# snphbaum/scikit-gpuppy

Hardware: AMD Instinct MI355X
Metric: GP fit+predict pts/sec (K+Cholesky, N=16384 d=8) (higher is better)
Workload: dtype f64; 1 GPU; C3: N=16384 d=8 M=16384 fit(Gram+Cholesky+alpha)+estimate_many, theta fixed; global_batch=32768, parallelism=1 GPU

## Files before the change

### scikit-gpuppy_amd/csrc/emu.hip

```cpp
#include <math.h>
#include <stdint.h>
#include <stdlib.h>
#include <algorithm>

#include "common.h"

#include "gemm_tile.h"

typedef int v4i __attribute__((ext_vector_type(4)));
typedef int v16i __attribute__((ext_vector_type(16)));

constexpr int EMU_MAXL = 16;
constexpr int EMU_BT = 256;
constexpr int EMU_BK = 128;

constexpr int EMU_MODULI[EMU_MAXL] = {256, 255, 253, 251, 247, 241, 239, 233, 229, 227, 223, 211, 199, 197, 193, 191};

struct EmuGarner { float c[EMU_MAXL][EMU_MAXL]; };
constexpr EmuGarner emu_garner_table()
{
    EmuGarner g{};
    for (int k = 0; k < EMU_MAXL; ++k)
        for (int j = 0; j < k; ++j) {
            const int pk = EMU_MODULI[k], a = EMU_MODULI[j] % pk;
            int inv = 0;
            for (int x = 1; x < pk; ++x)
                if (a * x % pk == 1) { inv = x; break; }
            g.c[j][k] = (float)inv;
        }
    return g;
}
static __constant__ const int emu_p[EMU_MAXL] = {256, 255, 253, 251, 247, 241, 239, 233, 229, 227, 223, 211, 199, 197, 193, 191};
static __constant__ const EmuGarner emu_garner = emu_garner_table();

constexpr int EMU_NONFINITE = 0x7fffffff;

int emu_moduli()
{
    static const int v = [] { const char *e = getenv("GPX_EMU_MODULI"); const int l = e ? atoi(e) : EMU_MAXL; return std::min(EMU_MAXL, std::max(2, l)); }();
    return v;
}
bool emu_enabled(int64_t K)
{
    static const int on = [] { const char *e = getenv("GPX_EMU_F64"); return e ? atoi(e) : 1; }();
    static const long min_k = [] { const char *e = getenv("GPX_EMU_MIN_K"); return e ? atol(e) : 4096L; }();
    return on && K >= min_k && K < (1 << 17) && K % EMU_BK == 0;
}
int emu_scale_bits(int64_t K, int L)
{
    double log2p = 0.0;
    for (int l = 0; l < L; ++l) log2p += log2((double)EMU_MODULI[l]);
    return (int)floor(log2p - 1.0 - log2((double)K) - 1e-9);
}

__global__ __launch_bounds__(256) void emu_split_kernel(const double *__restrict__ X, long ldx, long rows_real, int K, int bits, int L,
                                                        int8_t *__restrict__ res, long plane, int *__restrict__ sig)
{
    const long row = blockIdx.x;
    const int t = threadIdx.x;
    __shared__ double red_max[4];
    __shared__ int red_bad[4];
    int8_t *out = res + row * (long)K;
    if (row >= rows_real) {
        for (int c = 4 * t; c < K; c += 1024)
            for (int l = 0; l < L; ++l) *reinterpret_cast<int *>(out + l * plane + c) = 0;
        if (t == 0) sig[row] = 0;
        return;
    }
    const double *x = X + row * ldx;
    double m = 0.0;
    int bad = 0;
    for (int c = 2 * t; c < K; c += 512) {
        const v2d v = *reinterpret_cast<const v2d *>(x + c);
        bad |= (int)!isfinite(v.x) | (int)!isfinite(v.y);
        m = fmax(m, fmax(fabs(v.x), fabs(v.y)));
    }
#pragma unroll
    for (int o = 32; o > 0; o >>= 1) { m = fmax(m, __shfl_xor(m, o)); bad |= __shfl_xor(bad, o); }
    if ((t & 63) == 0) { red_max[t >> 6] = m; red_bad[t >> 6] = bad; }
    __syncthreads();
    m = fmax(fmax(red_max[0], red_max[1]), fmax(red_max[2], red_max[3]));
    bad = red_bad[0] | red_bad[1] | red_bad[2] | red_bad[3];
    const int s = (bad || m == 0.0) ? 0 : bits - 1 - ilogb(m);
    if (t == 0) sig[row] = bad ? EMU_NONFINITE : s;
    for (int c = 4 * t; c < K; c += 1024) {
        const v2d v0 = *reinterpret_cast<const v2d *>(x + c), v1 = *reinterpret_cast<const v2d *>(x + c + 2);
        double a[4] = {rint(ldexp(v0.x, s)), rint(ldexp(v0.y, s)), rint(ldexp(v1.x, s)), rint(ldexp(v1.y, s))};
        if (bad) a[0] = a[1] = a[2] = a[3] = 0.0;
#pragma unroll
        for (int l = 0; l < EMU_MAXL; ++l) {
            if (l >= L) continue;
            const double p = (double)emu_p[l], pinv = 1.0 / p, h = 0.5 * p;
            unsigned packed = 0;
#pragma unroll
            for (int e = 0; e < 4; ++e) {
                double r = fma(-rint(a[e] * pinv), p, a[e]);
                r = r > h ? r - p : (r < -h ? r + p : r);
                packed |= ((unsigned)(int)r & 0xffu) << (8 * e);
            }
            *reinterpret_cast<unsigned *>(out + l * plane + c) = packed;
        }
    }
}

__global__ __launch_bounds__(512, 1) void emu_i8_gemm_kernel(const int8_t *__restrict__ A, const int8_t *__restrict__ B, long sa, long sb, int K,
                                                             int8_t *__restrict__ R, long ldr, long sr, int tm, int tn)
{
    __shared__ __attribute__((aligned(1024))) int8_t smem[2 * 2 * EMU_BT * EMU_BK];
    constexpr int STAGE = 2 * EMU_BT * EMU_BK;
    const int nwg = gridDim.x, orig = blockIdx.x;
    const int lid = xcd_chunk_start(nwg, orig & 7) + (orig >> 3);
    const int per = tm * tn, z = lid / per;
    int rem = lid - z * per;
    const int g = rem / (8 * tn), first = 8 * g, grows = std::min(8, tm - first);
    rem -= g * 8 * tn;
    const int bx = rem / grows, by = first + rem - bx * grows;

    const int t = threadIdx.x;
    const int wave = __builtin_amdgcn_readfirstlane(t >> 6), lane = t & 63;
    const int wr = wave >> 2, wc = wave & 3;
    const int drow = lane >> 3;
    const char *Abase = reinterpret_cast<const char *>(A + z * sa + (long)by * EMU_BT * K);
    const char *Bbase = reinterpret_cast<const char *>(B + z * sb + (long)bx * EMU_BT * K);
    unsigned off[4];
#pragma unroll
    for (int u = 0; u < 4; ++u) {
        const int row = 8 * (wave + 8 * u) + drow;
        off[u] = (unsigned)((long)row * K + 16 * ((lane & 7) ^ ((row >> 1) & 7)));
    }
    const unsigned lds_base = (unsigned)(unsigned long)(__attribute__((address_space(3))) int8_t *)smem;
#define EMU_DMA_ONE(SBASE, VOFF, LDSBYTES) \
    asm volatile("s_mov_b32 m0, %0\n\ts_nop 0\n\tglobal_load_lds_dwordx4 %1, %2" ::"s"(LDSBYTES), "v"(VOFF), "s"(SBASE) : "memory");
#define EMU_DMA_STAGE(BUF, KT)                                                                                              \
    {                                                                                                                       \
        const char *ak_ = gpx_uniform_ptr(Abase + (long)(KT) * EMU_BK);                                                     \
        const char *bk_ = gpx_uniform_ptr(Bbase + (long)(KT) * EMU_BK);                                                     \
        _Pragma("unroll") for (int u_ = 0; u_ < 4; ++u_)                                                                    \
            EMU_DMA_ONE(ak_, off[u_], __builtin_amdgcn_readfirstlane(lds_base + (unsigned)((BUF) * STAGE + (wave + 8 * u_) * 1024)))  \
        _Pragma("unroll") for (int u_ = 0; u_ < 4; ++u_)                                                                    \
            EMU_DMA_ONE(bk_, off[u_], __builtin_amdgcn_readfirstlane(lds_base + (unsigned)((BUF) * STAGE + EMU_BT * EMU_BK + (wave + 8 * u_) * 1024))) \
    }
    const int nk = K / EMU_BK;
    EMU_DMA_STAGE(0, 0)
    v16i acc[4][2];
#pragma unroll
    for (int i = 0; i < 4; ++i)
#pragma unroll
        for (int j = 0; j < 2; ++j) acc[i][j] = (v16i){};
    asm volatile("s_waitcnt vmcnt(0)" ::: "memory");
    __syncthreads();

    const int fr = lane & 31, sw = (fr >> 1) & 7;
    int koff[4];
#pragma unroll
    for (int kk = 0; kk < 4; ++kk) koff[kk] = 16 * ((2 * kk + (lane >> 5)) ^ sw);
    const int a_row = (wr * 128 + fr) * EMU_BK, b_row = EMU_BT * EMU_BK + (wc * 64 + fr) * EMU_BK;
    typedef const __attribute__((address_space(3))) v4i lds_v4i;
    const __attribute__((address_space(3))) int8_t *lsm = (const __attribute__((address_space(3))) int8_t *)smem;
    v4i fa[2][4], fb[2][2];
#define EMU_LOAD_FRAGS(SET, BUFOFF, KK)                                                              \
    _Pragma("unroll") for (int i_ = 0; i_ < 4; ++i_)                                                 \
        fa[SET][i_] = *(lds_v4i *)(lsm + (BUFOFF) + a_row + i_ * 32 * EMU_BK + koff[KK]);            \
    _Pragma("unroll") for (int i_ = 0; i_ < 2; ++i_)                                                 \
        fb[SET][i_] = *(lds_v4i *)(lsm + (BUFOFF) + b_row + i_ * 32 * EMU_BK + koff[KK]);
#define EMU_MMA(SET)                                                                                 \
    _Pragma("unroll") for (int i_ = 0; i_ < 4; ++i_)                                                 \
        _Pragma("unroll") for (int j_ = 0; j_ < 2; ++j_)                                             \
            acc[i_][j_] = __builtin_amdgcn_mfma_i32_32x32x32_i8(fa[SET][i_], fb[SET][j_], acc[i_][j_], 0, 0, 0);
    EMU_LOAD_FRAGS(0, 0, 0)
#define EMU_KSTEP(CUR_OFF, NXT_OFF, NXT_BUF, KT)                   \
    {                                                             \
        const bool has_next_ = (KT) + 1 < nk;                     \
        if (has_next_) EMU_DMA_STAGE(NXT_BUF, (KT) + 1)           \
        EMU_LOAD_FRAGS(1, CUR_OFF, 1)                             \
        EMU_MMA(0)                                                \
        __builtin_amdgcn_sched_barrier(0);                        \
        EMU_LOAD_FRAGS(0, CUR_OFF, 2)                             \
        EMU_MMA(1)                                                \
        __builtin_amdgcn_sched_barrier(0);                        \
        EMU_LOAD_FRAGS(1, CUR_OFF, 3)                             \
        EMU_MMA(0)                                                \
        __builtin_amdgcn_sched_barrier(0);                        \
        asm volatile("s_waitcnt vmcnt(0)" ::: "memory");          \
        __syncthreads();                                          \
        if (has_next_) { EMU_LOAD_FRAGS(0, NXT_OFF, 0) }          \
        EMU_MMA(1)                                                \
        __builtin_amdgcn_sched_barrier(0);                        \
    }
    for (int kt = 0; kt < nk; kt += 2) {
        EMU_KSTEP(0, STAGE, 1, kt)
        if (kt + 1 < nk) EMU_KSTEP(STAGE, 0, 0, kt + 1)
    }
#undef EMU_KSTEP
#undef EMU_LOAD_FRAGS
#undef EMU_MMA
#undef EMU_DMA_STAGE
#undef EMU_DMA_ONE

    const double p = (double)emu_p[z], pinv = 1.0 / p;
    int8_t *Rw = R + z * sr + ((long)by * EMU_BT + wr * 128 + 4 * (lane >> 5)) * ldr + (long)bx * EMU_BT + wc * 64 + fr;
#pragma unroll
    for (int i = 0; i < 4; ++i)
#pragma unroll
        for (int j = 0; j < 2; ++j)
#pragma unroll
            for (int r = 0; r < 16; ++r) {
                const double v = (double)acc[i][j][r];
                Rw[(long)(i * 32 + (r & 3) + 8 * (r >> 2)) * ldr + j * 32] = (int8_t)(int)fma(-rint(v * pinv), p, v);
            }
}

__global__ __launch_bounds__(256) void emu_rebuild_kernel(const int8_t *__restrict__ R, long ldr, long sr, int L, const int *__restrict__ sa,
                                                          const int *__restrict__ sb, double *__restrict__ C, long ldc, long rows, long cols)
{
    const long q4 = (cols + 3) >> 2;
    const long idx = (long)blockIdx.x * 256 + threadIdx.x;
    const long i = idx / q4, j0 = (idx - i * q4) * 4;
    if (i >= rows) return;
    unsigned w[EMU_MAXL];
#pragma unroll
    for (int l = 0; l < EMU_MAXL; ++l)
        if (l < L) w[l] = *reinterpret_cast<const unsigned *>(R + l * sr + i * ldr + j0);
    const int si = sa[i];
    double *c = C + i * ldc + j0;
#pragma unroll
    for (int e = 0; e < 4; ++e) {
        if (j0 + e >= cols) continue;
        const int tj = sb[j0 + e];
        if (si == EMU_NONFINITE || tj == EMU_NONFINITE) { c[e] = __builtin_nan(""); continue; }
        float v[EMU_MAXL];
        v[0] = (float)(int8_t)(w[0] >> (8 * e));
#pragma unroll
        for (int k = 1; k < EMU_MAXL; ++k) {
            if (k >= L) continue;
            const float pk = (float)emu_p[k], pkinv = 1.0f / pk, hk = 0.5f * (pk - 1.0f);
            float tk = (float)(int8_t)(w[k] >> (8 * e));
#pragma unroll
            for (int jj = 0; jj < k; ++jj) {
                tk = (tk - v[jj]) * emu_garner.c[jj][k];
                tk = fmaf(-rintf(tk * pkinv), pk, tk);
            }
            tk = tk > hk ? tk - pk : (tk < -hk ? tk + pk : tk);
            v[k] = tk;
        }
        __int128 X = (__int128)(int)v[L - 1];
#pragma unroll
        for (int k = EMU_MAXL - 2; k >= 0; --k)
            if (k <= L - 2) X = X * emu_p[k] + (int)v[k];
        const long hi = (long)(X >> 64);
        const unsigned long lo = (unsigned long)X;
        const double xd = (hi == ((long)lo >> 63)) ? (double)(long)lo : fma((double)hi, 0x1p64, (double)lo);
        c[e] -= ldexp(xd, -(si + tj));
    }
}

static int64_t emu_cap(int64_t K, int L) { return std::max<int64_t>(EMU_BT, (((int64_t)1 << 31) / (K * L)) / EMU_BT * EMU_BT); }

void emu_work_need(EmuWork &w, int64_t rows, int64_t cols, int64_t K)
{
    const int L = emu_moduli();
    const int64_t cap = emu_cap(K, L), rt = std::min(round_up(rows, EMU_BT), cap), ct = std::min(round_up(cols, EMU_BT), cap);
    w.a_bytes = std::max(w.a_bytes, rt * K * L);
    w.b_bytes = std::max(w.b_bytes, ct * K * L);
    w.r_bytes = std::max(w.r_bytes, std::min(rt * ct * L, (int64_t)1 << 31));
    w.sig_n = std::max(w.sig_n, rt + ct);
}

int emu_work_alloc(EmuWork &w)
{
    double *a = nullptr, *b = nullptr, *r = nullptr, *g = nullptr;
    int rc = 0;
    if ((rc = dalloc(&a, w.a_bytes / 8)) || (rc = dalloc(&b, w.b_bytes / 8)) || (rc = dalloc(&r, w.r_bytes / 8)) || (rc = dalloc(&g, (w.sig_n + 1) / 2))) {
        if (a) dfree(a);
        if (b) dfree(b);
        if (r) dfree(r);
        return rc;
    }
    w.ra = (int8_t *)a;
    w.rb = (int8_t *)b;
    w.rr = (int8_t *)r;
    w.sig = (int *)g;
    return 0;
}

void emu_work_free(EmuWork &w)
{
    if (w.ra) dfree(w.ra);
    if (w.rb) dfree(w.rb);
    if (w.rr) dfree(w.rr);
    if (w.sig) dfree(w.sig);
    w = EmuWork();
}

static int emu_check_args(const double *A, int64_t lda, const double *B, int64_t ldb, int64_t ldc, int64_t cols, int64_t K)
{
    if (K <= 0 || K % EMU_BK || K >= (1 << 17)) {
        gpx_set_error("emu_gemm_nt_sub: K = %ld is not a multiple of %d in [%d, 2^17)", (long)K, EMU_BK, EMU_BK);
        return GPX_ERR_BAD_ARG;
    }
    if (lda < K || ldb < K || ldc < cols) {
        gpx_set_error("emu_gemm_nt_sub: leading dimension shorter than a row (lda %ld, ldb %ld < K %ld, or ldc %ld < cols %ld)", (long)lda, (long)ldb,
                      (long)K, (long)ldc, (long)cols);
        return GPX_ERR_BAD_ARG;
    }
    if ((lda | ldb) & 1 || ((uintptr_t)A | (uintptr_t)B) & 15) {
        gpx_set_error("emu_gemm_nt_sub: A and B must be 16-byte aligned with even lda, ldb (lda %ld, ldb %ld, A %p, B %p)", (long)lda, (long)ldb,
                      (const void *)A, (const void *)B);
        return GPX_ERR_BAD_ARG;
    }
    return 0;
}

int emu_gemm_nt_sub(const double *A, int64_t lda, const double *B, int64_t ldb, double *C, int64_t ldc, int64_t rows, int64_t cols, int64_t K,
                    const EmuWork &w, hipStream_t s, Profiler *prof)
{
    if (rows <= 0 || cols <= 0) return 0;
    if (K % EMU_BK || K >= (1 << 17)) { gpx_set_error("emu_gemm_nt_sub: K = %ld out of range", (long)K); return GPX_ERR_BAD_ARG; }
    const int L = emu_moduli();
    const int bits = emu_scale_bits(K, L), abits = bits - bits / 2, bbits = bits / 2;
    const int64_t cap = emu_cap(K, L);
    const int64_t rt = std::min<int64_t>(round_up(rows, EMU_BT), cap);
    int64_t ct = std::min<int64_t>(round_up(cols, EMU_BT), cap);
    while (ct > EMU_BT && rt * ct * L > ((int64_t)1 << 31)) ct -= EMU_BT;
    if (!w.ra || rt * K * L > w.a_bytes || ct * K * L > w.b_bytes || rt * ct * L > w.r_bytes || rt + ct > w.sig_n) {
        gpx_set_error("emu_gemm_nt_sub: workspace too small for %ld x %ld x %ld", (long)rows, (long)cols, (long)K);
        return GPX_ERR_STATE;
    }
    ProfScope ps(prof, s, GPX_K_GEMM_EMU, 2.0 * (double)rows * (double)cols * (double)K);
    int8_t *ra = w.ra, *rb = w.rb, *rr = w.rr;
    int *sga = w.sig, *sgb = sga + rt;
    for (int64_t r0 = 0; r0 < rows; r0 += rt) {
        const int64_t nr = std::min(rt, rows - r0), nrp = round_up(nr, EMU_BT);
        hipLaunchKernelGGL(emu_split_kernel, dim3((unsigned)nrp), dim3(256), 0, s, A + r0 * lda, (long)lda, (long)nr, (int)K, abits, L, ra,
                           (long)(nrp * K), sga);
        for (int64_t c0 = 0; c0 < cols; c0 += ct) {
            const int64_t nc = std::min(ct, cols - c0), ncp = round_up(nc, EMU_BT);
            hipLaunchKernelGGL(emu_split_kernel, dim3((unsigned)ncp), dim3(256), 0, s, B + c0 * ldb, (long)ldb, (long)nc, (int)K, bbits, L, rb,
                               (long)(ncp * K), sgb);
            const int tm = (int)(nrp / EMU_BT), tn = (int)(ncp / EMU_BT);
            hipLaunchKernelGGL(emu_i8_gemm_kernel, dim3((unsigned)(tm * tn * L)), dim3(512), 0, s, (const int8_t *)ra, (const int8_t *)rb,
                               (long)(nrp * K), (long)(ncp * K), (int)K, rr, (long)ncp, (long)(nrp * ncp), tm, tn);
            const long thr = (long)nr * ((nc + 3) / 4);
            hipLaunchKernelGGL(emu_rebuild_kernel, dim3((unsigned)((thr + 255) / 256)), dim3(256), 0, s, (const int8_t *)rr, (long)ncp,
                               (long)(nrp * ncp), L, (const int *)sga, (const int *)sgb, C + r0 * ldc + c0, (long)ldc, (long)nr, (long)nc);
        }
        GPX_HIP(hipGetLastError());
    }
    return 0;
}

extern "C" int gpx_emu_gemm_nt_sub(const double *A, int64_t lda, const double *B, int64_t ldb, double *C, int64_t ldc, int64_t rows, int64_t cols,
                                   int64_t K)
{
    GPX_TRY(gpx_require_device());
    if (rows < 0 || cols < 0 || !A || !B || !C) { gpx_set_error("gpx_emu_gemm_nt_sub: bad arguments"); return GPX_ERR_BAD_ARG; }
    GPX_TRY(emu_check_args(A, lda, B, ldb, ldc, cols, K));
    if (rows == 0 || cols == 0) return 0;
    EmuWork w;
    emu_work_need(w, rows, cols, K);
    GPX_TRY(emu_work_alloc(w));
    int rc = emu_gemm_nt_sub(A, lda, B, ldb, C, ldc, rows, cols, K, w, 0, nullptr);
    if (hipStreamSynchronize(0) != hipSuccess && rc == 0) { gpx_set_error("gpx_emu_gemm_nt_sub: stream failed"); rc = GPX_ERR_HIP; }
    emu_work_free(w);
    return rc;
}

__global__ void emu_fill_kernel(int8_t *p, long n, unsigned seed)
{
    for (long i = (long)blockIdx.x * 256 + threadIdx.x; i < n; i += (long)gridDim.x * 256) {
        unsigned x = (unsigned)i * 2654435761u ^ seed;
        x ^= x >> 15; x *= 2246822519u; x ^= x >> 13;
        p[i] = (int8_t)(x & 0xff);
    }
}

extern "C" int gpx_bench_emu_i8(int64_t rows, int64_t cols, int64_t K, int nmod, int iters, double *ms)
{
    GPX_TRY(gpx_require_device());
    if (rows % EMU_BT || cols % EMU_BT || K % EMU_BK || K >= (1 << 17) || nmod < 1 || nmod > EMU_MAXL || iters < 1 || !ms) {
        gpx_set_error("gpx_bench_emu_i8: bad arguments");
        return GPX_ERR_BAD_ARG;
    }
    double *wa = nullptr, *wb = nullptr, *wr = nullptr;
    int rc = 0;
    if ((rc = dalloc(&wa, rows * K * nmod / 8)) || (rc = dalloc(&wb, cols * K * nmod / 8)) || (rc = dalloc(&wr, rows * cols * nmod / 8))) {
        if (wa) dfree(wa);
        if (wb) dfree(wb);
        return rc;
    }
    hipLaunchKernelGGL(emu_fill_kernel, dim3(4096), dim3(256), 0, 0, (int8_t *)wa, (long)(rows * K * nmod), 1u);
    hipLaunchKernelGGL(emu_fill_kernel, dim3(4096), dim3(256), 0, 0, (int8_t *)wb, (long)(cols * K * nmod), 2u);
    const int tm = (int)(rows / EMU_BT), tn = (int)(cols / EMU_BT);
    hipEvent_t e0 = nullptr, e1 = nullptr;
    float t = 0.0f;
    hipError_t e = hipEventCreate(&e0);
    if (e == hipSuccess) e = hipEventCreate(&e1);
    for (int it = -1; it < iters && e == hipSuccess; ++it) {
        if (it == 0) e = hipEventRecord(e0, 0);
        hipLaunchKernelGGL(emu_i8_gemm_kernel, dim3((unsigned)(tm * tn * nmod)), dim3(512), 0, 0, (const int8_t *)wa, (const int8_t *)wb,
                           (long)(rows * K), (long)(cols * K), (int)K, (int8_t *)wr, (long)cols, (long)(rows * cols), tm, tn);
        if (e == hipSuccess) e = hipGetLastError();
    }
    if (e == hipSuccess) e = hipEventRecord(e1, 0);
    if (e == hipSuccess) e = hipEventSynchronize(e1);
    if (e == hipSuccess) e = hipEventElapsedTime(&t, e0, e1);
    if (e != hipSuccess) { gpx_set_error("gpx_bench_emu_i8: %s", hipGetErrorString(e)); rc = GPX_ERR_HIP; }
    *ms = t / iters;
    if (e0) (void)hipEventDestroy(e0);
    if (e1) (void)hipEventDestroy(e1);
    (void)hipDeviceSynchronize();
    dfree(wa);
    dfree(wb);
    dfree(wr);
    return rc;
}
```

Before: 431,000 pts/s.

## Rework emulated-f64 split and CRT rebuild with fp32 limb reduction and summed CRT

The split kernel now stages each row through shared memory and reduces every scaled integer to residues with fp32 arithmetic over 14-bit limbs and precomputed per-modulus constants, replacing a per-modulus f64 reduction. The rebuild kernel replaces sequential Garner reconstruction with a direct CRT weighted sum kept in 18-bit integer limbs using mul24, followed by a single quotient correction. It also transposes results through shared memory so stores to C are coalesced, with a vectorised variant when C is aligned. The aim is to cut ALU cost and uncoalesced traffic in the pre- and post-processing around the int8 GEMM that emulates f64. The cost is more shared memory per block and more delicate exact-arithmetic bookkeeping that must stay correct for every modulus count.

Result: faster. 443,900 pts/s (median of 6 runs) (+3.0%).

```diff
diff --git a/scikit-gpuppy_amd/csrc/emu.hip b/scikit-gpuppy_amd/csrc/emu.hip
--- a/scikit-gpuppy_amd/csrc/emu.hip
+++ b/scikit-gpuppy_amd/csrc/emu.hip
@@ -16,22 +16,59 @@
 
 constexpr int EMU_MODULI[EMU_MAXL] = {256, 255, 253, 251, 247, 241, 239, 233, 229, 227, 223, 211, 199, 197, 193, 191};
 
-struct EmuGarner { float c[EMU_MAXL][EMU_MAXL]; };
-constexpr EmuGarner emu_garner_table()
-{
-    EmuGarner g{};
-    for (int k = 0; k < EMU_MAXL; ++k)
-        for (int j = 0; j < k; ++j) {
-            const int pk = EMU_MODULI[k], a = EMU_MODULI[j] % pk;
-            int inv = 0;
-            for (int x = 1; x < pk; ++x)
-                if (a * x % pk == 1) { inv = x; break; }
-            g.c[j][k] = (float)inv;
-        }
-    return g;
-}
 static __constant__ const int emu_p[EMU_MAXL] = {256, 255, 253, 251, 247, 241, 239, 233, 229, 227, 223, 211, 199, 197, 193, 191};
-static __constant__ const EmuGarner emu_garner = emu_garner_table();
+
+struct EmuSplitTab { float c[EMU_MAXL][4], p[EMU_MAXL], pinv[EMU_MAXL]; };
+constexpr EmuSplitTab emu_split_table()
+{
+    EmuSplitTab t{};
+    for (int l = 0; l < EMU_MAXL; ++l) {
+        const int p = EMU_MODULI[l];
+        int r = 1;
+        for (int k = 0; k < 4; ++k) {
+            r = (int)(((long)r << 14) % p);
+            t.c[l][k] = (float)(r > p / 2 ? r - p : r);
+        }
+        t.p[l] = (float)p;
+        t.pinv[l] = 1.0f / (float)p;
+    }
+    return t;
+}
+static __constant__ const EmuSplitTab emu_split_tab = emu_split_table();
+
+constexpr int EMU_LIMBS = 7, EMU_LIMB_BITS = 18, EMU_Q_BITS = 19;
+struct EmuCrt {
+    int w[EMU_MAXL + 1][EMU_LIMBS + 1];
+    unsigned long p_lo, p_hi, h_lo, h_hi;
+};
+struct EmuCrtAll { EmuCrt t[EMU_MAXL + 1]; };
+constexpr EmuCrtAll emu_crt_table()
+{
+    EmuCrtAll a{};
+    for (int L = 2; L <= EMU_MAXL; ++L) {
+        EmuCrt &t = a.t[L];
+        unsigned __int128 P = 1;
+        for (int l = 0; l < L; ++l) P *= (unsigned)EMU_MODULI[l];
+        for (int l = 0; l < L; ++l) {
+            const unsigned p = (unsigned)EMU_MODULI[l];
+            const unsigned __int128 M = P / p;
+            const unsigned m = (unsigned)(M % p);
+            unsigned f = 0;
+            for (unsigned x = 1; x < p; ++x)
+                if (m * x % p == 1) { f = x; break; }
+            const unsigned __int128 W = M * f;
+            for (int k = 0; k < EMU_LIMBS; ++k) t.w[l][k] = (int)((W >> (EMU_LIMB_BITS * k)) & ((1u << EMU_LIMB_BITS) - 1));
+            t.w[l][EMU_LIMBS] = (int)((((unsigned long)f << EMU_Q_BITS) + p / 2) / p);
+        }
+        for (int k = 0; k < EMU_LIMBS; ++k) t.w[EMU_MAXL][k] = (int)((P >> (EMU_LIMB_BITS * k)) & ((1u << EMU_LIMB_BITS) - 1));
+        t.p_lo = (unsigned long)P;
+        t.p_hi = (unsigned long)(P >> 64);
+        t.h_lo = (unsigned long)(P >> 1);
+        t.h_hi = (unsigned long)(P >> 65);
+    }
+    return a;
+}
+static __constant__ const EmuCrtAll emu_crt = emu_crt_table();
 
 constexpr int EMU_NONFINITE = 0x7fffffff;
 
@@ -53,17 +90,21 @@
     return (int)floor(log2p - 1.0 - log2((double)K) - 1e-9);
 }
 
+constexpr int EMU_XROW = 18;
+typedef float v2f __attribute__((ext_vector_type(2)));
+
 __global__ __launch_bounds__(256) void emu_split_kernel(const double *__restrict__ X, long ldx, long rows_real, int K, int bits, int L,
                                                         int8_t *__restrict__ res, long plane, int *__restrict__ sig)
 {
     const long row = blockIdx.x;
-    const int t = threadIdx.x;
+    const int t = threadIdx.x, wave = t >> 6, lane = t & 63;
     __shared__ double red_max[4];
     __shared__ int red_bad[4];
+    __shared__ __attribute__((aligned(16))) double turn[256 * EMU_XROW];
     int8_t *out = res + row * (long)K;
     if (row >= rows_real) {
-        for (int c = 4 * t; c < K; c += 1024)
-            for (int l = 0; l < L; ++l) *reinterpret_cast<int *>(out + l * plane + c) = 0;
+        for (int c = 16 * t; c < K; c += 4096)
+            for (int l = 0; l < L; ++l) *reinterpret_cast<v4i *>(out + l * plane + c) = (v4i){};
         if (t == 0) sig[row] = 0;
         return;
     }
@@ -77,29 +118,68 @@
     }
 #pragma unroll
     for (int o = 32; o > 0; o >>= 1) { m = fmax(m, __shfl_xor(m, o)); bad |= __shfl_xor(bad, o); }
-    if ((t & 63) == 0) { red_max[t >> 6] = m; red_bad[t >> 6] = bad; }
+    if (lane == 0) { red_max[wave] = m; red_bad[wave] = bad; }
     __syncthreads();
     m = fmax(fmax(red_max[0], red_max[1]), fmax(red_max[2], red_max[3]));
     bad = red_bad[0] | red_bad[1] | red_bad[2] | red_bad[3];
     const int s = (bad || m == 0.0) ? 0 : bits - 1 - ilogb(m);
     if (t == 0) sig[row] = bad ? EMU_NONFINITE : s;
-    for (int c = 4 * t; c < K; c += 1024) {
-        const v2d v0 = *reinterpret_cast<const v2d *>(x + c), v1 = *reinterpret_cast<const v2d *>(x + c + 2);
-        double a[4] = {rint(ldexp(v0.x, s)), rint(ldexp(v0.y, s)), rint(ldexp(v1.x, s)), rint(ldexp(v1.y, s))};
-        if (bad) a[0] = a[1] = a[2] = a[3] = 0.0;
-#pragma unroll
-        for (int l = 0; l < EMU_MAXL; ++l) {
-            if (l >= L) continue;
-            const double p = (double)emu_p[l], pinv = 1.0 / p, h = 0.5 * p;
-            unsigned packed = 0;
-#pragma unroll
-            for (int e = 0; e < 4; ++e) {
-                double r = fma(-rint(a[e] * pinv), p, a[e]);
-                r = r > h ? r - p : (r < -h ? r + p : r);
-                packed |= ((unsigned)(int)r & 0xffu) << (8 * e);
+    for (int c0 = 0; c0 < K; c0 += 4096) {
+#pragma unroll
+        for (int e = 0; e < 8; ++e) {
+            const int col = c0 + 1024 * wave + 128 * e + 2 * lane;
+            v2d v = (v2d){0.0, 0.0};
+            if (col < K) v = *reinterpret_cast<const v2d *>(x + col);
+            *reinterpret_cast<v2d *>(turn + (64 * wave + 8 * e + (lane >> 3)) * EMU_XROW + 2 * (lane & 7)) = v;
+        }
+        __syncthreads();
+        const int c = c0 + 16 * t;
+        if (c < K) {
+            v2f h[8][5];
+#pragma unroll
+            for (int e = 0; e < 8; ++e) {
+                const v2d v = *reinterpret_cast<const v2d *>(turn + t * EMU_XROW + 2 * e);
+#pragma unroll
+                for (int u = 0; u < 2; ++u) {
+                    double a = bad ? 0.0 : rint(ldexp(u ? v.y : v.x, s));
+                    const double h4 = rint(a * 0x1p-56);
+                    a = fma(-h4, 0x1p56, a);
+                    const double h3 = rint(a * 0x1p-42);
+                    a = fma(-h3, 0x1p42, a);
+                    const double h2 = rint(a * 0x1p-28);
+                    a = fma(-h2, 0x1p28, a);
+                    const double h1 = rint(a * 0x1p-14);
+                    a = fma(-h1, 0x1p14, a);
+                    h[e][0][u] = (float)a;
+                    h[e][1][u] = (float)h1;
+                    h[e][2][u] = (float)h2;
+                    h[e][3][u] = (float)h3;
+                    h[e][4][u] = (float)h4;
+                }
             }
-            *reinterpret_cast<unsigned *>(out + l * plane + c) = packed;
-        }
+#pragma unroll
+            for (int l = 0; l < EMU_MAXL; ++l) {
+                if (l >= L) continue;
+                const float c1 = emu_split_tab.c[l][0], c2 = emu_split_tab.c[l][1], c3 = emu_split_tab.c[l][2], c4 = emu_split_tab.c[l][3];
+                const float p = emu_split_tab.p[l], pinv = emu_split_tab.pinv[l];
+                unsigned w[8];
+#pragma unroll
+                for (int e = 0; e < 8; ++e) {
+                    v2f sm = h[e][0] + h[e][1] * c1;
+                    sm = sm + h[e][2] * c2;
+                    sm = sm + h[e][3] * c3;
+                    sm = sm + h[e][4] * c4;
+                    const v2f q = __builtin_elementwise_rint(sm * pinv);
+                    const v2f r = (sm - q * p) + 12582912.0f;
+                    w[e] = __builtin_amdgcn_perm(__float_as_uint(r.y), __float_as_uint(r.x), 0x0c0c0400u);
+                }
+                v4i o;
+#pragma unroll
+                for (int d = 0; d < 4; ++d) o[d] = (int)__builtin_amdgcn_perm(w[2 * d + 1], w[2 * d], 0x05040100u);
+                *reinterpret_cast<v4i *>(out + l * plane + c) = o;
+            }
+        }
+        __syncthreads();
     }
 }
 
@@ -210,47 +290,115 @@
             }
 }
 
+constexpr int EMU_RROW = 10;
+typedef int v2i __attribute__((ext_vector_type(2)));
+
+template <bool WIDE>
 __global__ __launch_bounds__(256) void emu_rebuild_kernel(const int8_t *__restrict__ R, long ldr, long sr, int L, const int *__restrict__ sa,
-                                                          const int *__restrict__ sb, double *__restrict__ C, long ldc, long rows, long cols)
-{
-    const long q4 = (cols + 3) >> 2;
-    const long idx = (long)blockIdx.x * 256 + threadIdx.x;
-    const long i = idx / q4, j0 = (idx - i * q4) * 4;
-    if (i >= rows) return;
-    unsigned w[EMU_MAXL];
-#pragma unroll
-    for (int l = 0; l < EMU_MAXL; ++l)
-        if (l < L) w[l] = *reinterpret_cast<const unsigned *>(R + l * sr + i * ldr + j0);
+                                                          const int *__restrict__ sb, double *__restrict__ C, long ldc, long rows, long cols,
+                                                          long chunks)
+{
+    __shared__ __attribute__((aligned(16))) double turn[256 * EMU_RROW];
+    __shared__ __attribute__((aligned(16))) int ltab[EMU_MAXL + 1][EMU_LIMBS + 1];
+    const int t = threadIdx.x, wave = t >> 6, lane = t & 63;
+    if (t < (EMU_MAXL + 1) * (EMU_LIMBS + 1)) ltab[t >> 3][t & 7] = emu_crt.t[L].w[t >> 3][t & 7];
+    __syncthreads();
+    const long unit = (long)blockIdx.x * 4 + wave;
+    const long i = unit / chunks, cbase = (unit - i * chunks) * 512;
+    const bool live = i < rows;
+    const long j0 = cbase + 8 * lane;
+    if (live && j0 < cols) {
+        const int8_t *rp = R + i * ldr + j0;
+        v2i w[4];
+#pragma unroll
+        for (int u = 0; u < 4; ++u) {
+            w[u] = (v2i){};
+            if (u < L) w[u] = *reinterpret_cast<const v2i *>(rp + u * sr);
+        }
+        int S[8][EMU_LIMBS + 1];
+#pragma unroll
+        for (int e = 0; e < 8; ++e)
+#pragma unroll
+            for (int k = 0; k <= EMU_LIMBS; ++k) S[e][k] = 0;
+#pragma unroll 1
+        for (int l = 0; l < L; ++l) {
+            v2i wn = (v2i){};
+            if (l + 4 < L) wn = *reinterpret_cast<const v2i *>(rp + (l + 4) * sr);
+            const v4i wa = *reinterpret_cast<const v4i *>(&ltab[l][0]), wb = *reinterpret_cast<const v4i *>(&ltab[l][4]);
+            const int wl[EMU_LIMBS + 1] = {wa[0], wa[1], wa[2], wa[3], wb[0], wb[1], wb[2], wb[3]};
+#pragma unroll
+            for (int e = 0; e < 8; ++e) {
+                const int r = (int)(int8_t)(w[0][e >> 2] >> (8 * (e & 3)));
+#pragma unroll
+                for (int k = 0; k <= EMU_LIMBS; ++k) S[e][k] += __mul24(r, wl[k]);
+            }
+            w[0] = w[1];
+            w[1] = w[2];
+            w[2] = w[3];
+            w[3] = wn;
+        }
+        const EmuCrt &tab = emu_crt.t[L];
+        const v4i wa = *reinterpret_cast<const v4i *>(&ltab[EMU_MAXL][0]), wb = *reinterpret_cast<const v4i *>(&ltab[EMU_MAXL][4]);
+        const int pl[EMU_LIMBS + 1] = {wa[0], wa[1], wa[2], wa[3], wb[0], wb[1], wb[2], wb[3]};
+        const __int128 P = (__int128)(((unsigned __int128)tab.p_hi << 64) | tab.p_lo);
+        const __int128 H = (__int128)(((unsigned __int128)tab.h_hi << 64) | tab.h_lo);
+        double xd[8];
+#pragma unroll
+        for (int e = 0; e < 8; ++e) {
+            const int nq = -((S[e][EMU_LIMBS] + (1 << (EMU_Q_BITS - 1))) >> EMU_Q_BITS);
+            int T[EMU_LIMBS];
+#pragma unroll
+            for (int k = 0; k < EMU_LIMBS; ++k) T[k] = S[e][k] + __mul24(nq, pl[k]);
+#pragma unroll
+            for (int k = 0; k + 1 < EMU_LIMBS; ++k) {
+                T[k + 1] += T[k] >> EMU_LIMB_BITS;
+                T[k] &= (1 << EMU_LIMB_BITS) - 1;
+            }
+            const unsigned long xlo = (unsigned long)T[0] | ((unsigned long)T[1] << 18) | ((unsigned long)T[2] << 36) | ((unsigned long)T[3] << 54);
+            const unsigned long xhi = (unsigned long)(T[3] >> 10) | ((unsigned long)T[4] << 8) | ((unsigned long)T[5] << 26) |
+                                      ((unsigned long)(long)T[6] << 44);
+            __int128 X = (__int128)(((unsigned __int128)xhi << 64) | xlo);
+            X = X >= H ? X - P : (X < -H ? X + P : X);
+            const long hi = (long)(X >> 64);
+            const unsigned long lo = (unsigned long)X;
+            xd[e] = (hi == ((long)lo >> 63)) ? (double)(long)lo : fma((double)hi, 0x1p64, (double)lo);
+        }
+#pragma unroll
+        for (int e = 0; e < 8; e += 2) *reinterpret_cast<v2d *>(turn + t * EMU_RROW + e) = (v2d){xd[e], xd[e + 1]};
+    }
+    __syncthreads();
+    if (!live) return;
     const int si = sa[i];
-    double *c = C + i * ldc + j0;
-#pragma unroll
-    for (int e = 0; e < 4; ++e) {
-        if (j0 + e >= cols) continue;
-        const int tj = sb[j0 + e];
-        if (si == EMU_NONFINITE || tj == EMU_NONFINITE) { c[e] = __builtin_nan(""); continue; }
-        float v[EMU_MAXL];
-        v[0] = (float)(int8_t)(w[0] >> (8 * e));
-#pragma unroll
-        for (int k = 1; k < EMU_MAXL; ++k) {
-            if (k >= L) continue;
-            const float pk = (float)emu_p[k], pkinv = 1.0f / pk, hk = 0.5f * (pk - 1.0f);
-            float tk = (float)(int8_t)(w[k] >> (8 * e));
-#pragma unroll
-            for (int jj = 0; jj < k; ++jj) {
-                tk = (tk - v[jj]) * emu_garner.c[jj][k];
-                tk = fmaf(-rintf(tk * pkinv), pk, tk);
+    double *c = C + i * ldc;
+    const double *mine = turn + 64 * wave * EMU_RROW;
+    if (WIDE) {
+#pragma unroll
+        for (int e = 0; e < 4; ++e) {
+            const int n = 128 * e + 2 * lane;
+            const long j = cbase + n;
+            if (j >= cols) continue;
+            const v2d x = *reinterpret_cast<const v2d *>(mine + (n >> 3) * EMU_RROW + (n & 7));
+            const int t0 = sb[j], t1 = sb[j + 1];
+            const bool n0 = si == EMU_NONFINITE || t0 == EMU_NONFINITE, n1 = si == EMU_NONFINITE || t1 == EMU_NONFINITE;
+            if (j + 1 < cols) {
+                v2d v = *reinterpret_cast<v2d *>(c + j);
+                v.x = n0 ? __builtin_nan("") : v.x - ldexp(x.x, -(si + t0));
+                v.y = n1 ? __builtin_nan("") : v.y - ldexp(x.y, -(si + t1));
+                *reinterpret_cast<v2d *>(c + j) = v;
+            } else {
+                c[j] = n0 ? __builtin_nan("") : c[j] - ldexp(x.x, -(si + t0));
             }
-            tk = tk > hk ? tk - pk : (tk < -hk ? tk + pk : tk);
-            v[k] = tk;
-        }
-        __int128 X = (__int128)(int)v[L - 1];
-#pragma unroll
-        for (int k = EMU_MAXL - 2; k >= 0; --k)
-            if (k <= L - 2) X = X * emu_p[k] + (int)v[k];
-        const long hi = (long)(X >> 64);
-        const unsigned long lo = (unsigned long)X;
-        const double xd = (hi == ((long)lo >> 63)) ? (double)(long)lo : fma((double)hi, 0x1p64, (double)lo);
-        c[e] -= ldexp(xd, -(si + tj));
+        }
+    } else {
+#pragma unroll
+        for (int e = 0; e < 8; ++e) {
+            const int n = 64 * e + lane;
+            const long j = cbase + n;
+            if (j >= cols) continue;
+            const double x = mine[(n >> 3) * EMU_RROW + (n & 7)];
+            const int tj = sb[j];
+            c[j] = (si == EMU_NONFINITE || tj == EMU_NONFINITE) ? __builtin_nan("") : c[j] - ldexp(x, -(si + tj));
+        }
     }
 }
 
@@ -340,9 +488,15 @@
             const int tm = (int)(nrp / EMU_BT), tn = (int)(ncp / EMU_BT);
             hipLaunchKernelGGL(emu_i8_gemm_kernel, dim3((unsigned)(tm * tn * L)), dim3(512), 0, s, (const int8_t *)ra, (const int8_t *)rb,
                                (long)(nrp * K), (long)(ncp * K), (int)K, rr, (long)ncp, (long)(nrp * ncp), tm, tn);
-            const long thr = (long)nr * ((nc + 3) / 4);
-            hipLaunchKernelGGL(emu_rebuild_kernel, dim3((unsigned)((thr + 255) / 256)), dim3(256), 0, s, (const int8_t *)rr, (long)ncp,
-                               (long)(nrp * ncp), L, (const int *)sga, (const int *)sgb, C + r0 * ldc + c0, (long)ldc, (long)nr, (long)nc);
+            const long chunks = (nc + 511) / 512;
+            const unsigned rgrid = (unsigned)((nr * chunks + 3) / 4);
+            double *c = C + r0 * ldc + c0;
+            if (((uintptr_t)c & 15) == 0 && ldc % 2 == 0)
+                hipLaunchKernelGGL(emu_rebuild_kernel<true>, dim3(rgrid), dim3(256), 0, s, (const int8_t *)rr, (long)ncp, (long)(nrp * ncp), L,
+                                   (const int *)sga, (const int *)sgb, c, (long)ldc, (long)nr, (long)nc, chunks);
+            else
+                hipLaunchKernelGGL(emu_rebuild_kernel<false>, dim3(rgrid), dim3(256), 0, s, (const int8_t *)rr, (long)ncp, (long)(nrp * ncp), L,
+                                   (const int *)sga, (const int *)sgb, c, (long)ldc, (long)nr, (long)nc, chunks);
         }
         GPX_HIP(hipGetLastError());
     }
```
